# adeebkor/fenicsx-fus

Hardware: AMD Instinct MI355X
Metric: DOF-updates/sec (RK4 step) at p=4 hex fp64 (higher is better)
Workload: dtype f64; 1 GPU; 3D homogeneous wave, hex p=4 f64, Linear RK4, weak scaling: 64^3 cells per GPU (BASELINE.json configs[1]); ndofs_global=16974593, cells_per_gpu=262144, medium=water, partition=x-slabs x1, transport=none, blocks=8192, mfma_contractions=False, mfma_4x4x4_index1=False, packed_fp32=False, lds_bytes_per_block=72504

## Files before the change

fenicsx-fus_amd/csrc/fusmi.hip:

```cpp
#include "../../include/fusmi.h"

#include <dlfcn.h>
#include <hip/hip_runtime.h>
#include <rccl/rccl.h>
#include <limits>

#include <algorithm>
#include <cmath>
#include <cstdio>
#include <cstring>
#include <atomic>
#include <map>
#include <mutex>
#include <tuple>
#include <memory>
#include <string>
#include <vector>

#include "kernels.hpp"
#include "layout.hpp"
#include "tables.hpp"

using namespace fus;

// ... 221 lines not shown
  *p = q;
  return FUS_OK;
}
template <typename U>
static int upload(std::vector<void*>& pool, U** p, const std::vector<U>& v, hipStream_t st)
{
  FUSCHK(dalloc(pool, p, v.size()));
  if (!v.empty())
    HIPCHK(hipMemcpyAsync(*p, v.data(), v.size() * sizeof(U), hipMemcpyHostToDevice, st));
  return FUS_OK;
}
static inline unsigned nblk(int64_t n, int bs = 256) { return (unsigned)((n + bs - 1) / bs); }

struct ProfScope
{
  fus_ctx* c;
  Prof* p = nullptr;
  hipEvent_t e0 = nullptr, e1 = nullptr;
  ProfScope(fus_ctx* c_, const char* name) : c(c_)
  {
    bool take = c->prof == 1;
    if (c->prof == 2 && !strncmp(name, "stiffness", 9))
      take = (c->profs[name].seen++ % c->prof_sample) == 0;
    if (take)
    {
      p = &c->profs[name];
      (void)hipEventCreate(&e0), (void)hipEventCreate(&e1);
      (void)hipEventRecord(e0, c->stream);
    }
  }
  ~ProfScope()
  {
    if (p)
    {
      (void)hipEventRecord(e1, c->stream);
      p->ev.emplace_back(e0, e1);
    }
  }
};

template <typename T, int P, int OP, int ATOMIC, int STAGE, int NF, int GEOM, int TD = 3, int MF = 0, int PK = 0>
static int launch_block_op_v(fus_op* op, const T* geo, const T* coef, const T* x, T* bvec,
                             const StageArgs<T>& S, int blk_begin, int blk_count)
{
  if (blk_count <= 0)
    return FUS_OK;
  constexpr int N = P + 1;
  KArgs<T, N> K;
  for (int i = 0; i < N * N; ++i)
    K.Dk.d[i] = (T)op->D[i], K.Dk.dt[i] = (T)op->D[(i % N) * N + i / N];

  for (int i = 0; i < N; ++i)
    K.Dk.w[i] = (T)op->wts[i], K.Dk.x[i] = (T)op->nodes[i];
  static std::atomic<uint64_t> attr_set{0};
  const uint64_t dev_bit = 1ull << (op->ctx->device & 63);
  if (!(attr_set.load(std::memory_order_relaxed) & dev_bit))
  {
    HIPCHK(hipFuncSetAttribute(reinterpret_cast<const void*>(&k_block_op<T, P, OP, ATOMIC, STAGE, NF, GEOM, TD, MF, PK>),
                               hipFuncAttributeMaxDynamicSharedMemorySize, 160 * 1024));
    attr_set.fetch_or(dev_bit, std::memory_order_relaxed);
  }
  K.A = op->A;
  if (GEOM == GEOM_DIAG)
  {
    for (int q = 0; q < N; ++q)
      for (int i = 0; i < N; ++i)
      {
        double acc = 0;
        for (int m = 0; m < N; ++m)
          acc += op->D[m * N + q] * op->wts[m] * op->D[m * N + i];
        K.Dk.d[q * N + i] = K.Dk.dt[q * N + i] = (T)acc;
      }
  }
  K.A.blk_begin = blk_begin;
  K.A.blk_count = blk_count;
  K.Dg = static_cast<const T*>(op->d_Dg), K.geo = geo, K.coef = coef, K.x = x, K.bvec = bvec;
  K.partial = static_cast<T*>(op->d_partial);
  K.S = S;
  int grid = blk_count;
  if (GEOM != GEOM_STREAM && TD == 3 && op->ctx->walk != 0)
  {
    int per_cu = op->ctx->walk;
    if (per_cu < 0)
    {
      static std::mutex occ_mu;
      static std::map<std::tuple<int, int, size_t>, int> occ_cache;
      int occ = 0;
      {
        std::lock_guard<std::mutex> lk(occ_mu);
        const auto key = std::make_tuple(op->ctx->device, op->L.waves, op->lds_bytes);
        auto it = occ_cache.find(key);
        if (it == occ_cache.end())
        {
          int nb = 0;
          HIPCHK(hipOccupancyMaxActiveBlocksPerMultiprocessor(
              &nb, reinterpret_cast<const void*>(&k_block_op<T, P, OP, ATOMIC, STAGE, NF, GEOM, TD, MF, PK>), 64 * op->L.waves,
              op->lds_bytes));
          it = occ_cache.emplace(key, std::max(nb, 1)).first;
        }
        occ = it->second;
      }
      per_cu = (blk_count >= 4 * occ * op->ctx->num_cus) ? occ : 0;
    }
    if (per_cu > 0)
      grid = std::min(blk_count, per_cu * op->ctx->num_cus);
  }
  hipLaunchKernelGGL((k_block_op<T, P, OP, ATOMIC, STAGE, NF, GEOM, TD, MF, PK>), dim3(grid),
                     dim3(64 * op->L.waves), op->lds_bytes, op->ctx->stream, K);
  HIPCHK(hipGetLastError());
  return FUS_OK;
}

template <typename T, int P, int OP, int STAGE, int NF = 1>
static int launch_block_op(fus_op* op, const T* geo, const T* coef, const T* x, T* bvec,
                           const StageArgs<T>& S, int blk_begin = 0, int blk_count = -1)
{
  if (NF > op->nfields)
    return fail(FUS_ERR_STATE, "operator data was not created for two-field models (option fields=2)");
  if (blk_count < 0)
    blk_count = op->L.nblocks - blk_begin;
  const int b0 = blk_begin, nb = blk_count;
  if constexpr (P >= 8)
  {
    if (op->tdim == 2)
      return op->deterministic
                 ? launch_block_op_v<T, P, OP, 0, STAGE, NF, GEOM_STREAM, 2>(op, geo, coef, x, bvec, S, b0, nb)
                 : launch_block_op_v<T, P, OP, 1, STAGE, NF, GEOM_STREAM, 2>(op, geo, coef, x, bvec, S, b0, nb);
    if (!(op->affine || op->trilinear))
      return op->deterministic
                 ? launch_block_op_v<T, P, OP, 0, STAGE, NF, GEOM_STREAM>(op, geo, coef, x, bvec, S, b0, nb)
                 : launch_block_op_v<T, P, OP, 1, STAGE, NF, GEOM_STREAM>(op, geo, coef, x, bvec, S, b0, nb);
    const T* gc = static_cast<const T*>(op->d_Gc);
    if (op->affine)
      return op->deterministic
                 ? launch_block_op_v<T, P, OP, 0, STAGE, NF, GEOM_AFFINE>(op, gc, coef, x, bvec, S, b0, nb)
                 : launch_block_op_v<T, P, OP, 1, STAGE, NF, GEOM_AFFINE>(op, gc, coef, x, bvec, S, b0, nb);
    return op->deterministic
               ? launch_block_op_v<T, P, OP, 0, STAGE, NF, GEOM_TRILINEAR>(op, gc, coef, x, bvec, S, b0, nb)
               : launch_block_op_v<T, P, OP, 1, STAGE, NF, GEOM_TRILINEAR>(op, gc, coef, x, bvec, S, b0, nb);
  }
  else
  {
  if (op->tdim == 2)
    return op->deterministic
               ? launch_block_op_v<T, P, OP, 0, STAGE, NF, GEOM_STREAM, 2>(op, geo, coef, x, bvec, S, b0, nb)
               : launch_block_op_v<T, P, OP, 1, STAGE, NF, GEOM_STREAM, 2>(op, geo, coef, x, bvec, S, b0, nb);
  if constexpr ((P == 6 || P == 7) && OP == OP_STIFFNESS && (STAGE == STAGE_NONE || STAGE >= 3))
  {
    if (op->mfma && !op->deterministic && op->tdim == 3 && (op->affine || op->trilinear))
    {
      const T* gc = static_cast<const T*>(op->d_Gc);
      return op->affine ? launch_block_op_v<T, P, OP, 1, STAGE, NF, GEOM_AFFINE, 3, 1>(op, gc, coef, x, bvec, S, b0, nb)
                        : launch_block_op_v<T, P, OP, 1, STAGE, NF, GEOM_TRILINEAR, 3, 1>(op, gc, coef, x, bvec, S, b0, nb);
    }
  }
  if constexpr (sizeof(T) == 4 && P >= 5 && P <= 7 && OP == OP_STIFFNESS)
  {
    if (op->pk && !op->mfma && !op->deterministic && op->tdim == 3 && (op->affine || op->trilinear))
    {
      const T* gc = static_cast<const T*>(op->d_Gc);
      return op->affine ? launch_block_op_v<T, P, OP, 1, STAGE, NF, GEOM_AFFINE, 3, 0, 1>(op, gc, coef, x, bvec, S, b0, nb)
                        : launch_block_op_v<T, P, OP, 1, STAGE, NF, GEOM_TRILINEAR, 3, 0, 1>(op, gc, coef, x, bvec, S, b0, nb);
    }
// ... 2439 lines not shown
```

fenicsx-fus_amd/csrc/kernels.hpp:

```cpp
#pragma once
#include <hip/hip_runtime.h>
#include <stdint.h>

#include "geom.hpp"

namespace fus
{

struct ShapeDev
{
  int32_t nelem, nloc, nint, nrounds;
  int64_t rounds_off, ldm_off;
};

struct BlockArgs
{
  const int32_t* blk_shape;
  const ShapeDev* shapes;
  const int32_t* blk_elem_off;
  const int32_t* blk_int_off;
  const int64_t* blk_sh_off;
  const int32_t* sh_gidx;
  const int32_t* sh_ppos;
  const int16_t* rounds;
  const uint16_t* ldm;
  int32_t nblocks;
  int32_t blk_begin;
  int32_t blk_count;
  int32_t lds_nloc;
  int32_t lds_nelem;
  int32_t waves;
};

template <typename T>
struct StageArgs
{
  const T* minv;
  T *vn, *un, *u0, *v0, *u_, *v_;
  T adt, bdt, gval;
  T b0dt, pdt, third;
  const int32_t* blk_bnd_off;
  const int32_t* bnd_idx;
  const T* bnd_src;
  const T* bnd_abs;
  const T* x2;
  const T* coef2;
  const T* bnd_src2;
  T dgval;
  const T* m0;
  const T* mn1;
};

enum
{
  STAGE_NONE = -1
// ... 1937 lines not shown
    const T w = FUS_LD(vn), v = FUS_LD(v0), va = FUS_LD(u_), xs = FUS_LD(un);
    FUS_ST(un, xs + (w * adt - va * R.pdt));
    vnext = kv * adt + v;
    FUS_ST(v_, vnext);
  }
  else if (STAGE == 7)
  {
    const T w = FUS_LD(vn), v = FUS_LD(v0), va = FUS_LD(u_), vb = FUS_LD(v_), xs = FUS_LD(un);
    FUS_ST(u0, (xs - vb * R.pdt) + ((va + vb) * T(2) + (v + w)) * R.b0dt);
    vnext = kv * bdt + ((vb * T(2) + (va + w)) - v) * R.third;
    FUS_ST(v0, vnext);
  }
  else
  {
    const T w = FUS_LD(vn);
    FUS_ST(u_, w * bdt + FUS_LD(u_));
    FUS_ST(v_, kv * bdt + FUS_LD(v_));
    FUS_ST(un, w * adt + FUS_LD(u0));
    vnext = kv * adt + FUS_LD(v0);
    FUS_ST(vn, vnext);
  }
#undef FUS_LD
#undef FUS_ST
  return vnext;
}

template <typename T, int N>
struct KArgs
{
  BlockArgs A;
  DTab<T, N> Dk;
  const T* Dg;
  const T* geo;
  const T* coef;
  const T* x;
  T* bvec;
  T* partial;
  StageArgs<T> S;
};

template <typename T, int N>
__device__ __forceinline__ void load_stage_args(const KArgs<T, N> __attribute__((address_space(4))) * q, StageArgs<T>& S)
{
  S.minv = q->S.minv;
  S.vn = q->S.vn, S.un = q->S.un, S.u0 = q->S.u0, S.v0 = q->S.v0, S.u_ = q->S.u_, S.v_ = q->S.v_;
  S.adt = q->S.adt, S.bdt = q->S.bdt, S.gval = q->S.gval;
  S.b0dt = q->S.b0dt, S.pdt = q->S.pdt, S.third = q->S.third;
  S.blk_bnd_off = q->S.blk_bnd_off, S.bnd_idx = q->S.bnd_idx;
  S.bnd_src = q->S.bnd_src, S.bnd_abs = q->S.bnd_abs;
  S.x2 = q->S.x2, S.coef2 = q->S.coef2, S.bnd_src2 = q->S.bnd_src2, S.dgval = q->S.dgval;
  S.m0 = q->S.m0, S.mn1 = q->S.mn1;
}

template <typename T, int P, int OP, int ATOMIC, int STAGE, int NF, int GEOM, int TD = 3, int MF = 0, int PK = 0>
__global__ void __launch_bounds__((P <= 4) ? 512 : FUS_MID_THREADS, (P >= 8) ? FUS_HI_WAVES : (P <= 4 && is_aff(GEOM))
                                                            ? 4
                                                            : ((GEOM == GEOM_TRILINEAR || (is_aff(GEOM) && P <= 6)) ? FUS_TRI_WAVES_T(T, P) : (FUS_PF1(T, P, OP, ATOMIC, GEOM, TD) ? 2 : 1)))
k_block_op(const KArgs<T, P + 1> kernel_args)
{
  (void)kernel_args;
  static_assert(TD == 3 || GEOM == GEOM_STREAM, "quadrilaterals use the streamed geometry");
  typedef KArgs<T, P + 1> KArgsT;
  typedef DTab<T, P + 1> DTabT;
  static_assert(offsetof(KArgsT, Dk) == sizeof(BlockArgs) && offsetof(DTabT, dt) == sizeof(T) * ((P + 1) * (P + 1) + 2 * (P + 1)),
                "dtab_row reads the table at these kernarg offsets");
  constexpr int N = P + 1, N2 = N * N, Nd = (TD == 3) ? N * N * N : N * N;
  constexpr int EPW = (64 / N2) > 0 ? (64 / N2) : 1;
  constexpr int LPE = (N2 <= 64) ? 64 : 128;
  constexpr int SLOT = tile_slot_entries<T, N, TD>();
  static_assert(N2 <= 128, "degrees up to 10");
  static_assert(LPE == 64 || !MF, "degrees 8-10: no matrix-core variants");
  static_assert(!PK || (sizeof(T) == 4 && EPW == 1 && LPE == 64 && TD == 3 && OP == OP_STIFFNESS && ATOMIC && !MF
                        && GEOM != GEOM_STREAM),
                "packed path: fp32 stiffness, degrees 5-7, per-cell geometry, LDS-atomic accumulation");
  constexpr int EPS = PK ? 2 : 1;

  typedef const KArgs<T, N> __attribute__((address_space(4))) * KP;
#define FUS_KARGS(q)                                                                               \
  KP q = (KP)__builtin_amdgcn_kernarg_segment_ptr();                             \
  asm volatile("" : "+s"(q))
  constexpr int GCS = geom_cell_stride(GEOM);
  constexpr int AW = 8 / (int)sizeof(T);
  typedef double A2 __attribute__((ext_vector_type(2)));
  extern __shared__ __align__(16) unsigned char smem_raw[];
#define FUS_PHASE_LDS(q)                                                                           \
  const int lds_nloc = q->A.lds_nloc, lds_nelem = q->A.lds_nelem, nwaves = q->A.waves;             \
  const int slots = (nwaves * 64 / LPE) * EPW * EPS;                                               \
  T* x_l = reinterpret_cast<T*>(smem_raw);                                                         \
  double* y_l = reinterpret_cast<double*>(x_l + lds_nloc);  \
  T* x2_l = reinterpret_cast<T*>(y_l + lds_nloc);                 \
  T* scratch = x2_l + (NF == 2 ? lds_nloc : 0);                                                    \
  T* D_l = scratch + (size_t)slots * SLOT;        \
  T* cf_l = D_l + N2;                                              \
  T* cf2_l = cf_l + lds_nelem;                                                                     \
  T* gc_l = cf2_l + (NF == 2 ? lds_nelem : 0);  \
  T* w_l = gc_l + GCS * lds_nelem;   \
  T* pt_l = w_l + (N <= 8 ? 8 : 12);                                                               \
  uint16_t* ldm_l = reinterpret_cast<uint16_t*>(w_l + (GCS ? (N <= 8 ? 16 : 24) : 0));  \
  int16_t* rt_l = reinterpret_cast<int16_t*>(ldm_l + (size_t)lds_nelem * Nd);                      \
  (void)y_l, (void)x2_l, (void)scratch, (void)D_l, (void)cf_l, (void)cf2_l, (void)gc_l, (void)w_l, (void)pt_l,      \
      (void)ldm_l, (void)rt_l, (void)slots

  const int tid0 = threadIdx.x, nthr = blockDim.x;
#define FUS_TID()                                                                                  \
  int tid = tid0;                                                                                  \
  asm volatile("" : "+v"(tid))
#define FUS_LANE_COORDS(q)                                                                         \
  FUS_TID();                                                                                       \
  const int lane = tid % LPE, wave = tid / LPE;         \
  const int s = lane / N2, p = lane - s * N2;                                                      \
  const int b = p / N, c = p - b * N;                                                              \
  const bool active = s < EPW;                                                                     \
  const int myslot = (wave * EPW + (active ? s : 0)) * EPS;                                        \
                                \
  T* sA = reinterpret_cast<T*>(smem_raw) + (size_t)((NF == 2 ? 2 : 1) + AW) * q->A.lds_nloc         \
          + (size_t)myslot * SLOT;                                                                 \
  T* sB = sA

  struct Meta
  {
    ShapeDev sh;
    int elem_off, int_off;
    int64_t sh_off;
  };
  auto meta_of = [&](KP q, int bk) -> Meta
  {
    Meta M;
    M.sh = q->A.shapes[q->A.blk_shape[bk]];
    M.elem_off = q->A.blk_elem_off[bk];
    M.int_off = q->A.blk_int_off[bk];
    M.sh_off = q->A.blk_sh_off[bk];
    return M;
  };
  typedef T V2 __attribute__((ext_vector_type(2)));
  typedef uint32_t U4 __attribute__((ext_vector_type(4)));
  constexpr int UI = (P <= 3) ? 3 : ((P == 4) ? 2 : (P <= 6 ? 4 : (P == 7 ? FUS_UI_P7 : FUS_UI_HI))),
                US = (P <= 3) ? 4 : ((P == 4) ? 3 : (P <= 7 ? 5 : FUS_UI_HI)),
                UL = (P <= 3) ? 2 : ((P == 4) ? 1 : 4);
  struct PLoad
  {
    V2 xi[UI], xi2[UI];
    T xs[US], xs2[US];
    U4 lq[UL];
    T cfv, cf2v, gcv, gcv2, dgv, xtail, xtail2;
  };
  auto p_idx = [&](KP q, const Meta& M, bool enable, int (&gi)[US]) __attribute__((always_inline))
  {
    FUS_TID();
    const int nsh = M.sh.nloc - M.sh.nint;
    const int32_t* gix = q->A.sh_gidx + M.sh_off;
#pragma unroll
    for (int u = 0; u < US; ++u)
      gi[u] = (enable && tid + u * nthr < nsh) ? gix[tid + u * nthr] : -1;
  };
  auto p_load = [&](KP q, const Meta& M, PLoad& L, bool with_tables, bool enable, const int (&gi)[US])
      __attribute__((always_inline))
  {
    FUS_TID();
    const ShapeDev& sh = M.sh;
    const T* __restrict__ x = q->x;
    const T* __restrict__ x2 = (NF == 2) ? q->S.x2 : x;
    const T* __restrict__ coef = q->coef;
    const T* __restrict__ coef2 = (NF == 2) ? q->S.coef2 : coef;
    const T* __restrict__ geo = q->geo;
    const T* __restrict__ Dg = q->Dg;
    const V2* xg = reinterpret_cast<const V2*>(x + M.int_off);
    const V2* xg2 = reinterpret_cast<const V2*>(x2 + M.int_off);
    const int nvec = sh.nint >> 1;
    const int nsh = sh.nloc - sh.nint;
    const int32_t* gix = q->A.sh_gidx + M.sh_off;
    const int n16 = (sh.nelem * Nd * 2 + 15) >> 4;
    const U4* lsrc = reinterpret_cast<const U4*>(q->A.ldm + sh.ldm_off);
    const int ngc = sh.nelem * GCS;
#pragma unroll
    for (int u = 0; u < UI; ++u)
    {
      const bool ok = enable && tid + u * nthr < nvec;
      L.xi[u] = ok ? xg[tid + u * nthr] : V2(T(0));
      L.xi2[u] = (NF == 2 && ok) ? xg2[tid + u * nthr] : V2(T(0));
    }
#pragma unroll
    for (int u = 0; u < UL; ++u)
      L.lq[u] = (enable && tid + u * nthr < n16) ? lsrc[tid + u * nthr] : U4(0u);
    L.cfv = (enable && tid < sh.nelem) ? coef[M.elem_off + tid] : T(0);
    L.cf2v = (NF == 2 && enable && tid < sh.nelem) ? coef2[M.elem_off + tid] : T(0);
    L.gcv = (enable && tid < ngc) ? geo[(int64_t)M.elem_off * GCS + tid] : T(0);
    L.gcv2 = (GCS > 7 && enable && tid + nthr < ngc) ? geo[(int64_t)M.elem_off * GCS + tid + nthr] : T(0);
    L.dgv = (with_tables && enable && tid < N2 + 2 * N) ? Dg[tid] : T(0);
    L.xtail = (enable && tid == 0 && (sh.nint & 1)) ? x[M.int_off + sh.nint - 1] : T(0);
    L.xtail2 = (NF == 2 && enable && tid == 0 && (sh.nint & 1)) ? x2[M.int_off + sh.nint - 1] : T(0);
#pragma unroll
    for (int u = 0; u < US; ++u)
    {
      L.xs[u] = gi[u] >= 0 ? x[gi[u]] : T(0);
      L.xs2[u] = (NF == 2 && gi[u] >= 0) ? x2[gi[u]] : T(0);
    }
  };
  auto p_commit = [&](KP q, const Meta& M, const PLoad& L, bool with_tables) __attribute__((always_inline))
  {
    FUS_PHASE_LDS(q);
    FUS_TID();
    const ShapeDev& sh = M.sh;
    const T* __restrict__ x = q->x;
    const T* __restrict__ x2 = (NF == 2) ? q->S.x2 : x;
    const T* __restrict__ coef = q->coef;
    const T* __restrict__ coef2 = (NF == 2) ? q->S.coef2 : coef;
    const T* __restrict__ geo = q->geo;
    const T* __restrict__ Dg = q->Dg;
    const V2* xg = reinterpret_cast<const V2*>(x + M.int_off);
    const V2* xg2 = reinterpret_cast<const V2*>(x2 + M.int_off);
    const int nvec = sh.nint >> 1;
    const int nsh = sh.nloc - sh.nint;
    const int32_t* gix = q->A.sh_gidx + M.sh_off;
    const int n16 = (sh.nelem * Nd * 2 + 15) >> 4;
    const U4* lsrc = reinterpret_cast<const U4*>(q->A.ldm + sh.ldm_off);
    const int ngc = sh.nelem * GCS;
    for (int i = tid; i < (sh.nloc + 1) / 2; i += nthr)
      reinterpret_cast<A2*>(y_l)[i] = A2(0.0);
#pragma unroll
    for (int u = 0; u < UI; ++u)
      if (tid + u * nthr < nvec)
      {
        reinterpret_cast<V2*>(x_l)[tid + u * nthr] = L.xi[u];
        if (NF == 2)
          reinterpret_cast<V2*>(x2_l)[tid + u * nthr] = L.xi2[u];
      }
#pragma unroll
    for (int u = 0; u < UL; ++u)
      if (tid + u * nthr < n16)
        reinterpret_cast<U4*>(ldm_l)[tid + u * nthr] = L.lq[u];
    if (tid < sh.nelem)
    {
      cf_l[tid] = L.cfv;
      if (NF == 2)
        cf2_l[tid] = L.cf2v;
    }
    if (tid < ngc)
      gc_l[tid] = L.gcv;
    if (GCS > 7 && tid + nthr < ngc)
      gc_l[tid + nthr] = L.gcv2;
    if (with_tables)
    {
      if (tid < N2)
        D_l[tid] = L.dgv;
      if (GCS && tid >= N2 && tid < N2 + N)
        w_l[tid - N2] = L.dgv;
      if (GCS && tid >= N2 + N && tid < N2 + 2 * N)
        pt_l[tid - N2 - N] = L.dgv;
      for (int k = tid + nthr; k < N2 + 2 * N; k += nthr)
      {
        const T v = Dg[k];
        if (k < N2)
          D_l[k] = v;
        else if (GCS && k < N2 + N)
          w_l[k - N2] = v;
        else if (GCS)
          pt_l[k - N2 - N] = v;
      }
    }
    if (tid == 0 && (sh.nint & 1))
    {
      x_l[sh.nint - 1] = L.xtail;
      if (NF == 2)
        x2_l[sh.nint - 1] = L.xtail2;
    }
#pragma unroll
    for (int u = 0; u < US; ++u)
      if (tid + u * nthr < nsh)
      {
        x_l[sh.nint + tid + u * nthr] = L.xs[u];
        if (NF == 2)
          x2_l[sh.nint + tid + u * nthr] = L.xs2[u];
      }
    constexpr int UB = 8;
    for (int base = tid + UI * nthr; base < nvec; base += nthr * UB)
    {
      V2 v[UB], v2[UB];
#pragma unroll
      for (int u = 0; u < UB; ++u)
        if (base + u * nthr < nvec)
        {
          v[u] = xg[base + u * nthr];
          if (NF == 2)
            v2[u] = xg2[base + u * nthr];
        }
#pragma unroll
      for (int u = 0; u < UB; ++u)
        if (base + u * nthr < nvec)
        {
          reinterpret_cast<V2*>(x_l)[base + u * nthr] = v[u];
          if (NF == 2)
            reinterpret_cast<V2*>(x2_l)[base + u * nthr] = v2[u];
        }
    }
    for (int base = tid + US * nthr; base < nsh; base += nthr * UB)
    {
      int g[UB];
      T v[UB], v2[UB];
#pragma unroll
      for (int u = 0; u < UB; ++u)
        g[u] = (base + u * nthr < nsh) ? gix[base + u * nthr] : 0;
#pragma unroll
      for (int u = 0; u < UB; ++u)
      {
        v[u] = x[g[u]];
        if (NF == 2)
          v2[u] = x2[g[u]];
      }
#pragma unroll
      for (int u = 0; u < UB; ++u)
        if (base + u * nthr < nsh)
        {
          x_l[sh.nint + base + u * nthr] = v[u];
          if (NF == 2)
            x2_l[sh.nint + base + u * nthr] = v2[u];
        }
    }
    for (int base = tid + UL * nthr; base < n16; base += nthr * UB)
    {
      U4 q[UB];
#pragma unroll
      for (int u = 0; u < UB; ++u)
        if (base + u * nthr < n16)
          q[u] = lsrc[base + u * nthr];
#pragma unroll
      for (int u = 0; u < UB; ++u)
        if (base + u * nthr < n16)
          reinterpret_cast<U4*>(ldm_l)[base + u * nthr] = q[u];
    }
    for (int k = tid + nthr; k < sh.nelem; k += nthr)
    {
      cf_l[k] = coef[M.elem_off + k];
      if (NF == 2)
        cf2_l[k] = coef2[M.elem_off + k];
    }
    for (int k = tid + (GCS > 7 ? 2 : 1) * nthr; k < ngc; k += nthr)
      gc_l[k] = geo[(int64_t)M.elem_off * GCS + k];
    if (!ATOMIC)
      for (int k = tid; k < sh.nrounds * slots; k += nthr)
        rt_l[k] = q->A.rounds[sh.rounds_off + k];
  };

  FUS_KARGS(q0);
  const int blk_end = q0->A.blk_begin + q0->A.blk_count;
  const int blk_stride = gridDim.x;
  int wg = blockIdx.x;
  if (FUS_XCD_REMAP)
  {
    const int G = gridDim.x, q8 = G >> 3, r8 = G & 7, xc = wg & 7;
    wg = xc * q8 + (xc < r8 ? xc : r8) + (wg >> 3);
  }
  int blk = wg + q0->A.blk_begin;
  FUS_STAMP(blk, 0);
  ElemIn<T, N, OP, GEOM, TD> inA, inB;
  auto first_fetch = [&](KP q, const Meta& Mm) __attribute__((always_inline))
  {
    FUS_LANE_COORDS(q);
    (void)b, (void)c, (void)sA, (void)sB;
    const int slots = (q->A.waves * 64 / LPE) * EPW * EPS;
    const int nt0 = ATOMIC ? (Mm.sh.nelem + slots - 1) / slots : Mm.sh.nrounds;
    int e0 = -1;
    if (active && nt0 > 0)
      e0 = ATOMIC ? (myslot < Mm.sh.nelem ? myslot : -1) : (int)q->A.rounds[Mm.sh.rounds_off + myslot];
    elem_fetch<T, N, OP, GEOM, TD>(inA, e0, q->geo, Mm.elem_off, p);
  };
  PLoad L;
  {
    const Meta M0 = meta_of(q0, blk);
    first_fetch(q0, M0);
    int gi0[US];
    p_idx(q0, M0, true, gi0);
    p_load(q0, M0, L, true, true, gi0);
  }
  bool first = true;
  for (;;)
  {
  FUS_KARGS(qc);
  FUS_PHASE_LDS(qc);
  FUS_LANE_COORDS(qc);
  const Meta M = meta_of(qc, blk);
  const ShapeDev& sh = M.sh;
  const int elem_off = M.elem_off;
  const int ntrips = ATOMIC ? (sh.nelem + slots - 1) / slots : sh.nrounds;
  auto elem_of = [&](int r) -> int
  {
    if (!active || r >= ntrips)
      return -1;
    if (ATOMIC)
      return (r * slots + myslot < sh.nelem) ? r * slots + myslot : -1;
    return (int)rt_l[r * slots + myslot];
  };
#ifdef FUS_PROBE_PFREE
  if (first)
    p_commit(qc, M, L, true);
  else
  {
    FUS_TID();
    for (int i = tid; i < (M.sh.nloc + 1) / 2; i += nthr)
      reinterpret_cast<A2*>(y_l)[i] = A2(0.0);
  }
#else
  p_commit(qc, M, L, first);
#endif
  const int blk_next = blk + blk_stride;
  const bool has_next = blk_next < blk_end;
  constexpr bool IDX_EARLY = false;
  int gi_n[US];
  if constexpr (IDX_EARLY)
  {
    Meta Mi{};
    if (has_next)
      Mi = meta_of(qc, blk_next);
    p_idx(qc, Mi, has_next, gi_n);
  }
  __syncthreads();
  FUS_STAMP(blk, 1);
#ifdef FUS_STAGGER
  if (tid0 >= 256)
    __builtin_amdgcn_s_sleep(FUS_STAGGER);
#endif
  T Drb[N], Drc[N], Dcb[N], Dcc[N], w3[N];
  T wbc, pb, pc;
  {
#pragma unroll
    for (int j = 0; j < N; ++j)
    {
      constexpr bool inreg = (OP == OP_STIFFNESS) && !(FUS_PF1(T, P, OP, ATOMIC, GEOM, TD) && P >= 6)
                             && GEOM != GEOM_TRILINEAR && GEOM != GEOM_DIAG && !(is_aff(GEOM) && (P == 5 || P == 6)) && !MF;
      Drb[j] = inreg ? D_l[b * N + j] : T(0);
      Drc[j] = inreg ? D_l[c * N + j] : T(0);
      Dcb[j] = inreg ? D_l[j * N + b] : T(0);
      Dcc[j] = inreg ? D_l[j * N + c] : T(0);
    }
#pragma unroll
    for (int a = 0; a < N; ++a)
      w3[a] = (GEOM == GEOM_AFFINE) ? w_l[a] * w_l[b] * w_l[c] : T(0);
    wbc = (GEOM == GEOM_TRILINEAR || GEOM == GEOM_DIAG) ? w_l[b] * w_l[c] : T(0);
    pb = (GEOM == GEOM_TRILINEAR) ? pt_l[b] : T(0), pc = (GEOM == GEOM_TRILINEAR) ? pt_l[c] : T(0);
  }

  FUS_KARGS(qt);
  DTab<T, N> Dk;
  if constexpr (!dtab_by_rows<T, N>())
  {
#pragma unroll
    for (int i = 0; i < N * N; ++i)
      Dk.d[i] = qt->Dk.d[i];
  }
#pragma unroll
  for (int i = 0; i < N; ++i)
    Dk.w[i] = qt->Dk.w[i], Dk.x[i] = qt->Dk.x[i];
  const T* __restrict__ geo = qt->geo;
#define FUS_ELEM_COMPUTE(in)                                                                       \
  do                                                                                               \
  {                                                                                                \
    if constexpr (LPE == 128 && TD == 2)                                                           \
      elem_compute2d<T, N, OP, ATOMIC, NF, true>(in, Drb, Drc, Dcb, Dcc, x_l, y_l, sA, ldm_l,      \
                                                 cf_l, x2_l, cf2_l, p, b, c, s == 0);              \
// ... 28 lines not shown
    {
      int li[N];
      T F0[N], F1[N], F2[N];
      constexpr int DL = (P >= 6) ? 1 : 0;
      const bool act = elem_stiff_fwd<T, N, NF, DL>(inA, Dk, Drb, Drc, D_l, x_l, sA, ldm_l, cf_l, x2_l, cf2_l, p, b,
                                                    c, li, F0, F1, F2);
      elem_fetch<T, N, OP, GEOM, TD>(inA, elem_of(r + 1), geo, elem_off, p);
      if (act)
        elem_stiff_bwd<T, N, DL, ATOMIC>(Dk, Dcb, Dcc, D_l, y_l, sA, p, b, c, li, F0, F1, F2);
      if (!ATOMIC && nwaves > 1)
        __syncthreads();
    }
  }
  else
  for (int r = 0; r < ntrips; r += 2)
  {
    const bool has1 = r + 1 < ntrips;
    elem_fetch<T, N, OP, GEOM, TD>(inB, elem_of(r + 1), geo, elem_off, p);
    FUS_ELEM_COMPUTE(inA);
    if (r == 0)
      FUS_STAMP(blk, 5);
    if (r == 2)
      FUS_STAMP(blk, 7);
    if (!ATOMIC && nwaves > 1)
      __syncthreads();
    elem_fetch<T, N, OP, GEOM, TD>(inA, elem_of(r + 2), geo, elem_off, p);
    if (has1)
    {
      FUS_ELEM_COMPUTE(inB);
      if (r == 0)
        FUS_STAMP(blk, 6);
      if (!ATOMIC && nwaves > 1)
        __syncthreads();
    }
  }
#undef FUS_ELEM_COMPUTE
  {
  FUS_KARGS(qe);
  FUS_PHASE_LDS(qe);
  FUS_TID();
  const Meta M = meta_of(qe, blk);
  const ShapeDev& sh = M.sh;
  const int int_off = M.int_off;
  const int64_t sh_off = M.sh_off;
  StageArgs<T> S;
  load_stage_args<T, N>(qe, S);
  T* __restrict__ bvec = qe->bvec;
  T* __restrict__ partial = qe->partial;
  const int32_t* __restrict__ pp = qe->A.sh_ppos + sh_off;
  const int nsh = sh.nloc - sh.nint;
  int ppv[US];
#pragma unroll
  for (int u = 0; u < US; ++u)
    ppv[u] = (tid + u * nthr < nsh) ? pp[tid + u * nthr] : -1;

  const int nvec = sh.nint >> 1;
    constexpr bool EPI2 = (P <= 4) && (NF == 1);
    struct Epi
    {
      bool on;
      int i, o;
      V2 bv, mi, w, a0, b0, au, av, m1, m0v, us;
    };
    auto epi_load = [&](int i, Epi& E, int part) __attribute__((always_inline))
    {
      if (part != 2)
      {
      E.on = i < nvec;
      E.i = i, E.o = int_off + 2 * i;
      E.bv = E.mi = E.w = E.a0 = E.b0 = E.au = E.av = E.m1 = E.m0v = E.us = V2(T(0));
#ifdef FUS_PROBE_EFREE
      auto ld = [&](const T* ptr) -> V2 { return E.on ? V2(T(1)) + V2(T((uintptr_t)ptr & 7)) : V2(T(0)); };
#else
      auto ld = [&](const T* ptr) -> V2
      { return E.on ? __builtin_nontemporal_load(reinterpret_cast<const V2*>(ptr + E.o)) : V2(T(0)); };
#endif
      constexpr bool WV = NF == 2;
      if (STAGE == 0)
        E.a0 = ld(S.u0), E.b0 = ld(S.v0);
      else if (STAGE == 4)
        E.b0 = ld(S.v0);
      else
        E.w = ld(S.vn);
      if (WV && S.mn1)
        E.m1 = ld(S.mn1), E.m0v = ld(S.m0);
      else
        E.mi = ld(S.minv);
      if (STAGE == 3)
        E.au = ld(S.u_), E.av = ld(S.v_);
      else if (STAGE == 1)
        E.au = ld(S.u_), E.av = ld(S.v_), E.a0 = ld(S.u0), E.b0 = ld(S.v0);
      else if (STAGE == 5)
        E.b0 = ld(S.v0);
      else if (STAGE == 6)
        E.b0 = ld(S.v0), E.au = ld(S.u_);
      else if (STAGE == 7)
        E.b0 = ld(S.v0), E.au = ld(S.u_), E.av = ld(S.v_);
      }
      if (part != 1)
      {
        constexpr bool WV2 = NF == 2;
        const A2 a2 = E.on ? reinterpret_cast<const A2*>(y_l)[E.i] : A2(0.0);
        E.bv = V2{(T)a2[0], (T)a2[1]};
        if ((WV2 && S.mn1) || STAGE >= 4)
          E.us = E.on ? reinterpret_cast<const V2*>(x_l)[E.i] : V2(T(0));
      }
    };
    auto epi_store = [&](const Epi& E) __attribute__((always_inline))
    {
      if (!E.on)
        return;
      auto st = [&](T* ptr, V2 val) { __builtin_nontemporal_store(val, reinterpret_cast<V2*>(ptr + E.o)); };
      V2 kv;
      if (NF == 2 && S.mn1)
      {
        const V2 vs = stage_is_first(STAGE) ? E.b0 : E.w;
        kv = (E.bv - E.m1 * vs * vs) / (E.m0v + E.m1 * E.us);
      }
      else
        kv = E.bv * E.mi;
      if (STAGE == 0)
      {
        st(S.u_, E.b0 * S.bdt + E.a0);
        st(S.v_, kv * S.bdt + E.b0);
        st(S.un, E.b0 * S.adt + E.a0);
        st(S.vn, kv * S.adt + E.b0);
      }
      else if (STAGE == 4)
      {
        st(S.un, E.b0 * S.adt + E.us);
        st(S.v_, kv * S.adt + E.b0);
      }
      else if (STAGE == 3)
      {
        st(S.u0, E.w * S.bdt + E.au);
        st(S.v0, kv * S.bdt + E.av);
      }
      else if (STAGE == 5)
      {
        st(S.un, E.us + (E.w * S.adt - E.b0 * S.pdt));
        st(S.v_, kv * S.adt + E.b0);
      }
      else if (STAGE == 6)
      {
        st(S.un, E.us + (E.w * S.adt - E.au * S.pdt));
        st(S.v_, kv * S.adt + E.b0);
      }
      else if (STAGE == 7)
      {
        st(S.u0, (E.us - E.av * S.pdt) + ((E.au + E.av) * T(2) + (E.b0 + E.w)) * S.b0dt);
        st(S.v0, kv * S.bdt + ((E.av * T(2) + (E.au + E.w)) - E.b0) * S.third);
      }
      else
      {
        st(S.u_, E.w * S.bdt + E.au);
        st(S.v_, kv * S.bdt + E.av);
        st(S.un, E.w * S.adt + E.a0);
        st(S.vn, kv * S.adt + E.b0);
      }
    };
    constexpr int EPIU = EPI2 ? 2 : epiu_of<T>(P, GEOM, NF);
    constexpr bool EARLY = epi_early<T>(P);
    Epi Ef[EPIU];
    if (EARLY && STAGE != STAGE_NONE)
    {
#pragma unroll
      for (int u = 0; u < EPIU; ++u)
        epi_load(tid + u * nthr, Ef[u], 1);
    }
  __syncthreads();
  FUS_STAMP(blk, 2);

  {
    FUS_KARGS(qn);
    Meta Mn{};
    if (has_next)
      Mn = meta_of(qn, blk_next);
#ifdef FUS_PROBE_PFREE
    if constexpr (!IDX_EARLY)
      p_idx(qn, Mn, false, gi_n);
    p_load(qn, Mn, L, false, false, gi_n);
#else
    if constexpr (!IDX_EARLY)
      p_idx(qn, Mn, has_next, gi_n);
    p_load(qn, Mn, L, false, has_next, gi_n);
#endif
  }
  if (STAGE == STAGE_NONE)
  {
    V2* bg = reinterpret_cast<V2*>(bvec + int_off);
    for (int i = tid; i < nvec; i += nthr)
    {
      const A2 a2 = reinterpret_cast<const A2*>(y_l)[i];
      bg[i] = V2{(T)a2[0], (T)a2[1]};
    }
    if (tid == 0 && (sh.nint & 1))
      bvec[int_off + sh.nint - 1] = (T)y_l[sh.nint - 1];
  }
  else
  {
    const int k0 = S.blk_bnd_off[blk], k1 = S.blk_bnd_off[blk + 1];
    if (k1 > k0)
    {
      const T* vstage = stage_is_first(STAGE) ? S.v0 : S.vn;
      for (int k = k0 + tid; k < k1; k += nthr)
      {
        const int gi = S.bnd_idx[k];
        T add = S.gval * S.bnd_src[k] - S.bnd_abs[k] * vstage[gi];
        if (NF == 2)
          add += S.dgval * S.bnd_src2[k];
        y_l[gi - int_off] += add;
      }
      __syncthreads();
    }
    if (tid == 0 && (sh.nint & 1))
      (void)stage_update_dof<T, STAGE>((int64_t)int_off + sh.nint - 1, (T)y_l[sh.nint - 1], S.minv, S.vn, S.un, S.u0,
                                       S.v0, S.u_, S.v_, S.adt, S.bdt, (NF == 2) ? S.m0 : nullptr,
                                       (NF == 2) ? S.mn1 : nullptr, LeanRK<T>{S.b0dt, S.pdt, S.third});
#pragma unroll
    for (int u = 0; u < EPIU; ++u)
      epi_load(tid + u * nthr, Ef[u], EARLY ? 2 : 0);
#pragma unroll
    for (int u = 0; u < EPIU; ++u)
      epi_store(Ef[u]);
    for (int i = tid + EPIU * nthr; i < nvec; i += EPIU * nthr)
    {
      Epi E[EPIU];
#pragma unroll
      for (int u = 0; u < EPIU; ++u)
        epi_load(i + u * nthr, E[u], 0);
#pragma unroll
      for (int u = 0; u < EPIU; ++u)
        epi_store(E[u]);
    }
  }
#pragma unroll
  for (int u = 0; u < US; ++u)
    if (ppv[u] >= 0)
      partial[ppv[u]] = (T)y_l[sh.nint + tid + u * nthr];
  for (int k = tid + US * nthr; k < nsh; k += nthr)
    partial[pp[k]] = (T)y_l[sh.nint + k];
  }
  FUS_TRACE_END(blk);
  if (!has_next)
    break;
  __syncthreads();
  blk = blk_next;
  first = false;
  {
    FUS_KARGS(qf);
    const Meta Mf = meta_of(qf, blk);
    first_fetch(qf, Mf);
  }
  }
#undef FUS_KARGS
#undef FUS_LANE_COORDS
#undef FUS_PHASE_LDS
#undef FUS_TID
}


template <typename T, typename I>
__global__ void k_shared_reduce(int64_t s0, int64_t s1, const I* __restrict__ sh_ptr,
                                const I* __restrict__ sh_pairs, const T* __restrict__ partial,
                                T* __restrict__ bsh)
{
  const int64_t s = s0 + (int64_t)blockIdx.x * blockDim.x + threadIdx.x;
  if (s >= s1)
    return;
  T acc = T(0);
  for (I k = sh_ptr[s]; k < sh_ptr[s + 1]; ++k)
    acc += partial[sh_pairs[k]];
  bsh[s] = acc;
}

template <typename T>
struct BndNext
{
  int enabled;
  int32_t npairs;
  const T *srcw, *absw, *src2w;
  T gnext, dgnext;
  T* partial;
};

template <typename T>
__device__ __forceinline__ void boundary_next(const BndNext<T>& B, int32_t last_pair, T vnext)
{
  if (B.enabled && last_pair >= B.npairs)
  {
    const int32_t k = last_pair - B.npairs;
    T v = B.gnext * B.srcw[k] - B.absw[k] * vnext;
    if (B.src2w)
      v += B.dgnext * B.src2w[k];
    B.partial[last_pair] = v;
  }
}



constexpr int FUS_MAX_PLANES = 16;
struct PartialPlanes
{
  int32_t bnd0;
  int32_t cnt[FUS_MAX_PLANES];
  int32_t off[FUS_MAX_PLANES];
};

template <typename T, int STAGE>
__global__ void __launch_bounds__(256)
k_shared_stage_planes(int64_t n, const PartialPlanes PL, const uint64_t* __restrict__ bnd_mask,
// ... 401 lines not shown
```

Before: 13.90 billion DOF-updates/s.

## Add WALK template specialization to slim single-block kernel path

Adds a WALK template parameter to the block operator kernel and picks the walking (persistent, multi-block) variant only when the grid is smaller than the block count. The non-walking variant drops the next-block prefetch and the compiler barriers on the kernarg pointer and thread id. It also uses predicated loads with 32-bit offset addressing and wave-uniform guards on the tail loops. The aim is to cut register pressure, scalar and address arithmetic, and dead prefetch code when each workgroup handles one block. The cost is twice as many kernel instantiations and more complex load-guard logic.

```diff
diff --git a/fenicsx-fus_amd/csrc/fusmi.hip b/fenicsx-fus_amd/csrc/fusmi.hip
--- a/fenicsx-fus_amd/csrc/fusmi.hip
+++ b/fenicsx-fus_amd/csrc/fusmi.hip
@@ -297,14 +297,6 @@
 
   for (int i = 0; i < N; ++i)
     K.Dk.w[i] = (T)op->wts[i], K.Dk.x[i] = (T)op->nodes[i];
-  static std::atomic<uint64_t> attr_set{0};
-  const uint64_t dev_bit = 1ull << (op->ctx->device & 63);
-  if (!(attr_set.load(std::memory_order_relaxed) & dev_bit))
-  {
-    HIPCHK(hipFuncSetAttribute(reinterpret_cast<const void*>(&k_block_op<T, P, OP, ATOMIC, STAGE, NF, GEOM, TD, MF, PK>),
-                               hipFuncAttributeMaxDynamicSharedMemorySize, 160 * 1024));
-    attr_set.fetch_or(dev_bit, std::memory_order_relaxed);
-  }
   K.A = op->A;
   if (GEOM == GEOM_DIAG)
   {
@@ -322,8 +314,9 @@
   K.Dg = static_cast<const T*>(op->d_Dg), K.geo = geo, K.coef = coef, K.x = x, K.bvec = bvec;
   K.partial = static_cast<T*>(op->d_partial);
   K.S = S;
+  constexpr bool CAN_WALK = GEOM != GEOM_STREAM && TD == 3;
   int grid = blk_count;
-  if (GEOM != GEOM_STREAM && TD == 3 && op->ctx->walk != 0)
+  if (CAN_WALK && op->ctx->walk != 0)
   {
     int per_cu = op->ctx->walk;
     if (per_cu < 0)
@@ -339,8 +332,8 @@
         {
           int nb = 0;
           HIPCHK(hipOccupancyMaxActiveBlocksPerMultiprocessor(
-              &nb, reinterpret_cast<const void*>(&k_block_op<T, P, OP, ATOMIC, STAGE, NF, GEOM, TD, MF, PK>), 64 * op->L.waves,
-              op->lds_bytes));
+              &nb, reinterpret_cast<const void*>(&k_block_op<T, P, OP, ATOMIC, STAGE, NF, GEOM, TD, MF, PK, CAN_WALK ? 1 : 0>),
+              64 * op->L.waves, op->lds_bytes));
           it = occ_cache.emplace(key, std::max(nb, 1)).first;
         }
         occ = it->second;
@@ -350,10 +343,27 @@
     if (per_cu > 0)
       grid = std::min(blk_count, per_cu * op->ctx->num_cus);
   }
-  hipLaunchKernelGGL((k_block_op<T, P, OP, ATOMIC, STAGE, NF, GEOM, TD, MF, PK>), dim3(grid),
-                     dim3(64 * op->L.waves), op->lds_bytes, op->ctx->stream, K);
-  HIPCHK(hipGetLastError());
-  return FUS_OK;
+  auto launch = [&](auto walk) -> int
+  {
+    constexpr int WALK = decltype(walk)::value;
+    const auto kernel = &k_block_op<T, P, OP, ATOMIC, STAGE, NF, GEOM, TD, MF, PK, WALK>;
+    static std::atomic<uint64_t> attr_set{0};
+    const uint64_t dev_bit = 1ull << (op->ctx->device & 63);
+    if (!(attr_set.load(std::memory_order_relaxed) & dev_bit))
+    {
+      HIPCHK(hipFuncSetAttribute(reinterpret_cast<const void*>(kernel), hipFuncAttributeMaxDynamicSharedMemorySize,
+                                 160 * 1024));
+      attr_set.fetch_or(dev_bit, std::memory_order_relaxed);
+    }
+    hipLaunchKernelGGL((k_block_op<T, P, OP, ATOMIC, STAGE, NF, GEOM, TD, MF, PK, WALK>), dim3(grid),
+                       dim3(64 * op->L.waves), op->lds_bytes, op->ctx->stream, K);
+    HIPCHK(hipGetLastError());
+    return FUS_OK;
+  };
+  if constexpr (CAN_WALK)
+    if (grid < blk_count)
+      return launch(std::integral_constant<int, 1>{});
+  return launch(std::integral_constant<int, 0>{});
 }
 
 template <typename T, int P, int OP, int STAGE, int NF = 1>
diff --git a/fenicsx-fus_amd/csrc/kernels.hpp b/fenicsx-fus_amd/csrc/kernels.hpp
--- a/fenicsx-fus_amd/csrc/kernels.hpp
+++ b/fenicsx-fus_amd/csrc/kernels.hpp
@@ -1,6 +1,7 @@
 #pragma once
 #include <hip/hip_runtime.h>
 #include <stdint.h>
+#include <type_traits>
 
 #include "geom.hpp"
 
@@ -2044,7 +2045,7 @@
   S.m0 = q->S.m0, S.mn1 = q->S.mn1;
 }
 
-template <typename T, int P, int OP, int ATOMIC, int STAGE, int NF, int GEOM, int TD = 3, int MF = 0, int PK = 0>
+template <typename T, int P, int OP, int ATOMIC, int STAGE, int NF, int GEOM, int TD = 3, int MF = 0, int PK = 0, int WALK = 0>
 __global__ void __launch_bounds__((P <= 4) ? 512 : FUS_MID_THREADS, (P >= 8) ? FUS_HI_WAVES : (P <= 4 && is_aff(GEOM))
                                                             ? 4
                                                             : ((GEOM == GEOM_TRILINEAR || (is_aff(GEOM) && P <= 6)) ? FUS_TRI_WAVES_T(T, P) : (FUS_PF1(T, P, OP, ATOMIC, GEOM, TD) ? 2 : 1)))
@@ -2069,8 +2070,9 @@
 
   typedef const KArgs<T, N> __attribute__((address_space(4))) * KP;
 #define FUS_KARGS(q)                                                                               \
-  KP q = (KP)__builtin_amdgcn_kernarg_segment_ptr();                             \
-  asm volatile("" : "+s"(q))
+  KP q = (KP)__builtin_amdgcn_kernarg_segment_ptr();                                               \
+  if constexpr (WALK)                                                                              \
+    asm volatile("" : "+s"(q))
   constexpr int GCS = geom_cell_stride(GEOM);
   constexpr int AW = 8 / (int)sizeof(T);
   typedef double A2 __attribute__((ext_vector_type(2)));
@@ -2096,7 +2098,8 @@
   const int tid0 = threadIdx.x, nthr = blockDim.x;
 #define FUS_TID()                                                                                  \
   int tid = tid0;                                                                                  \
-  asm volatile("" : "+v"(tid))
+  if constexpr (WALK)                                                                              \
+    asm volatile("" : "+v"(tid))
 #define FUS_LANE_COORDS(q)                                                                         \
   FUS_TID();                                                                                       \
   const int lane = tid % LPE, wave = tid / LPE;         \
@@ -2115,8 +2118,11 @@
     int elem_off, int_off;
     int64_t sh_off;
   };
+  Meta Mone{};
   auto meta_of = [&](KP q, int bk) -> Meta
   {
+    if constexpr (!WALK)
+      return Mone;
     Meta M;
     M.sh = q->A.shapes[q->A.blk_shape[bk]];
     M.elem_off = q->A.blk_elem_off[bk];
@@ -2124,6 +2130,21 @@
     M.sh_off = q->A.blk_sh_off[bk];
     return M;
   };
+  auto at32 = [](auto* base, int i) -> auto&
+  {
+    typedef std::remove_reference_t<decltype(*base)> E;
+    typedef std::conditional_t<std::is_const_v<E>, const char, char> C;
+    return *reinterpret_cast<E*>(reinterpret_cast<C*>(base) + (uint32_t)i * (uint32_t)sizeof(E));
+  };
+#define FUS_UNIFORM(cond) (WALK || __builtin_amdgcn_readfirstlane((int)(cond)))
+#define FUS_STAGE_LD(dst, cond, expr, fill)                                                        \
+  do                                                                                               \
+  {                                                                                                \
+    if constexpr (WALK)                                                                            \
+      dst = (cond) ? (expr) : (fill);                                                              \
+    else if (cond)                                                                                 \
+      dst = (expr);                                                                                \
+  } while (0)
   typedef T V2 __attribute__((ext_vector_type(2)));
   typedef uint32_t U4 __attribute__((ext_vector_type(4)));
   constexpr int UI = (P <= 3) ? 3 : ((P == 4) ? 2 : (P <= 6 ? 4 : (P == 7 ? FUS_UI_P7 : FUS_UI_HI))),
@@ -2143,7 +2164,7 @@
     const int32_t* gix = q->A.sh_gidx + M.sh_off;
 #pragma unroll
     for (int u = 0; u < US; ++u)
-      gi[u] = (enable && tid + u * nthr < nsh) ? gix[tid + u * nthr] : -1;
+      FUS_STAGE_LD(gi[u], enable && tid + u * nthr < nsh, at32(gix, tid + u * nthr), -1);
   };
   auto p_load = [&](KP q, const Meta& M, PLoad& L, bool with_tables, bool enable, const int (&gi)[US])
       __attribute__((always_inline))
@@ -2168,24 +2189,28 @@
     for (int u = 0; u < UI; ++u)
     {
       const bool ok = enable && tid + u * nthr < nvec;
-      L.xi[u] = ok ? xg[tid + u * nthr] : V2(T(0));
-      L.xi2[u] = (NF == 2 && ok) ? xg2[tid + u * nthr] : V2(T(0));
+      FUS_STAGE_LD(L.xi[u], ok, at32(xg, tid + u * nthr), V2(T(0)));
+      FUS_STAGE_LD(L.xi2[u], NF == 2 && ok, at32(xg2, tid + u * nthr), V2(T(0)));
     }
 #pragma unroll
     for (int u = 0; u < UL; ++u)
-      L.lq[u] = (enable && tid + u * nthr < n16) ? lsrc[tid + u * nthr] : U4(0u);
-    L.cfv = (enable && tid < sh.nelem) ? coef[M.elem_off + tid] : T(0);
-    L.cf2v = (NF == 2 && enable && tid < sh.nelem) ? coef2[M.elem_off + tid] : T(0);
-    L.gcv = (enable && tid < ngc) ? geo[(int64_t)M.elem_off * GCS + tid] : T(0);
-    L.gcv2 = (GCS > 7 && enable && tid + nthr < ngc) ? geo[(int64_t)M.elem_off * GCS + tid + nthr] : T(0);
-    L.dgv = (with_tables && enable && tid < N2 + 2 * N) ? Dg[tid] : T(0);
-    L.xtail = (enable && tid == 0 && (sh.nint & 1)) ? x[M.int_off + sh.nint - 1] : T(0);
-    L.xtail2 = (NF == 2 && enable && tid == 0 && (sh.nint & 1)) ? x2[M.int_off + sh.nint - 1] : T(0);
+      FUS_STAGE_LD(L.lq[u], enable && tid + u * nthr < n16, at32(lsrc, tid + u * nthr), U4(0u));
+    const T* cfg = coef + M.elem_off;
+    const T* cfg2 = coef2 + M.elem_off;
+    const T* gcg = geo + (int64_t)M.elem_off * GCS;
+    FUS_STAGE_LD(L.cfv, enable && tid < sh.nelem, at32(cfg, tid), T(0));
+    FUS_STAGE_LD(L.cf2v, NF == 2 && enable && tid < sh.nelem, at32(cfg2, tid), T(0));
+    FUS_STAGE_LD(L.gcv, enable && tid < ngc, at32(gcg, tid), T(0));
+    FUS_STAGE_LD(L.gcv2, GCS > 7 && enable && tid + nthr < ngc, at32(gcg, tid + nthr), T(0));
+    FUS_STAGE_LD(L.dgv, with_tables && enable && tid < N2 + 2 * N, at32(Dg, tid), T(0));
+    FUS_STAGE_LD(L.xtail, enable && tid == 0 && (sh.nint & 1), x[M.int_off + sh.nint - 1], T(0));
+    FUS_STAGE_LD(L.xtail2, NF == 2 && enable && tid == 0 && (sh.nint & 1), x2[M.int_off + sh.nint - 1], T(0));
 #pragma unroll
     for (int u = 0; u < US; ++u)
     {
-      L.xs[u] = gi[u] >= 0 ? x[gi[u]] : T(0);
-      L.xs2[u] = (NF == 2 && gi[u] >= 0) ? x2[gi[u]] : T(0);
+      const bool oks = WALK ? gi[u] >= 0 : tid + u * nthr < nsh;
+      FUS_STAGE_LD(L.xs[u], oks, x[(uint32_t)gi[u]], T(0));
+      FUS_STAGE_LD(L.xs2[u], NF == 2 && oks, x2[(uint32_t)gi[u]], T(0));
     }
   };
   auto p_commit = [&](KP q, const Meta& M, const PLoad& L, bool with_tables) __attribute__((always_inline))
@@ -2239,6 +2264,7 @@
         w_l[tid - N2] = L.dgv;
       if (GCS && tid >= N2 + N && tid < N2 + 2 * N)
         pt_l[tid - N2 - N] = L.dgv;
+      if (FUS_UNIFORM(nthr < N2 + 2 * N))
       for (int k = tid + nthr; k < N2 + 2 * N; k += nthr)
       {
         const T v = Dg[k];
@@ -2265,6 +2291,7 @@
           x2_l[sh.nint + tid + u * nthr] = L.xs2[u];
       }
     constexpr int UB = 8;
+    if (FUS_UNIFORM(UI * nthr < nvec))
     for (int base = tid + UI * nthr; base < nvec; base += nthr * UB)
     {
       V2 v[UB], v2[UB];
@@ -2285,6 +2312,7 @@
             reinterpret_cast<V2*>(x2_l)[base + u * nthr] = v2[u];
         }
     }
+    if (FUS_UNIFORM(US * nthr < nsh))
     for (int base = tid + US * nthr; base < nsh; base += nthr * UB)
     {
       int g[UB];
@@ -2308,6 +2336,7 @@
             x2_l[sh.nint + base + u * nthr] = v2[u];
         }
     }
+    if (FUS_UNIFORM(UL * nthr < n16))
     for (int base = tid + UL * nthr; base < n16; base += nthr * UB)
     {
       U4 q[UB];
@@ -2320,12 +2349,14 @@
         if (base + u * nthr < n16)
           reinterpret_cast<U4*>(ldm_l)[base + u * nthr] = q[u];
     }
+    if (FUS_UNIFORM(nthr < sh.nelem))
     for (int k = tid + nthr; k < sh.nelem; k += nthr)
     {
       cf_l[k] = coef[M.elem_off + k];
       if (NF == 2)
         cf2_l[k] = coef2[M.elem_off + k];
     }
+    if (FUS_UNIFORM((GCS > 7 ? 2 : 1) * nthr < ngc))
     for (int k = tid + (GCS > 7 ? 2 : 1) * nthr; k < ngc; k += nthr)
       gc_l[k] = geo[(int64_t)M.elem_off * GCS + k];
     if (!ATOMIC)
@@ -2358,6 +2389,13 @@
   };
   PLoad L;
   {
+    if constexpr (!WALK)
+    {
+      Mone.sh = q0->A.shapes[q0->A.blk_shape[blk]];
+      Mone.elem_off = q0->A.blk_elem_off[blk];
+      Mone.int_off = q0->A.blk_int_off[blk];
+      Mone.sh_off = q0->A.blk_sh_off[blk];
+    }
     const Meta M0 = meta_of(q0, blk);
     first_fetch(q0, M0);
     int gi0[US];
@@ -2395,7 +2433,7 @@
   p_commit(qc, M, L, first);
 #endif
   const int blk_next = blk + blk_stride;
-  const bool has_next = blk_next < blk_end;
+  const bool has_next = WALK && blk_next < blk_end;
   constexpr bool IDX_EARLY = false;
   int gi_n[US];
   if constexpr (IDX_EARLY)
@@ -2530,14 +2568,14 @@
   int ppv[US];
 #pragma unroll
   for (int u = 0; u < US; ++u)
-    ppv[u] = (tid + u * nthr < nsh) ? pp[tid + u * nthr] : -1;
+    FUS_STAGE_LD(ppv[u], tid + u * nthr < nsh, at32(pp, tid + u * nthr), -1);
 
   const int nvec = sh.nint >> 1;
     constexpr bool EPI2 = (P <= 4) && (NF == 1);
     struct Epi
     {
       bool on;
-      int i, o;
+      int i;
       V2 bv, mi, w, a0, b0, au, av, m1, m0v, us;
     };
     auto epi_load = [&](int i, Epi& E, int part) __attribute__((always_inline))
@@ -2545,37 +2583,41 @@
       if (part != 2)
       {
       E.on = i < nvec;
-      E.i = i, E.o = int_off + 2 * i;
-      E.bv = E.mi = E.w = E.a0 = E.b0 = E.au = E.av = E.m1 = E.m0v = E.us = V2(T(0));
+      E.i = i;
+      if constexpr (WALK)
+        E.bv = E.mi = E.w = E.a0 = E.b0 = E.au = E.av = E.m1 = E.m0v = E.us = V2(T(0));
 #ifdef FUS_PROBE_EFREE
-      auto ld = [&](const T* ptr) -> V2 { return E.on ? V2(T(1)) + V2(T((uintptr_t)ptr & 7)) : V2(T(0)); };
+      auto ld = [&](V2& dst, const T* ptr) { dst = E.on ? V2(T(1)) + V2(T((uintptr_t)ptr & 7)) : V2(T(0)); };
 #else
-      auto ld = [&](const T* ptr) -> V2
-      { return E.on ? __builtin_nontemporal_load(reinterpret_cast<const V2*>(ptr + E.o)) : V2(T(0)); };
+      auto ld = [&](V2& dst, const T* ptr)
+      {
+        FUS_STAGE_LD(dst, E.on, __builtin_nontemporal_load(&at32(reinterpret_cast<const V2*>(ptr + int_off), E.i)),
+                     V2(T(0)));
+      };
 #endif
       constexpr bool WV = NF == 2;
       if (STAGE == 0)
-        E.a0 = ld(S.u0), E.b0 = ld(S.v0);
+        ld(E.a0, S.u0), ld(E.b0, S.v0);
       else if (STAGE == 4)
-        E.b0 = ld(S.v0);
+        ld(E.b0, S.v0);
       else
-        E.w = ld(S.vn);
+        ld(E.w, S.vn);
       if (WV && S.mn1)
-        E.m1 = ld(S.mn1), E.m0v = ld(S.m0);
+        ld(E.m1, S.mn1), ld(E.m0v, S.m0);
       else
-        E.mi = ld(S.minv);
+        ld(E.mi, S.minv);
       if (STAGE == 3)
-        E.au = ld(S.u_), E.av = ld(S.v_);
+        ld(E.au, S.u_), ld(E.av, S.v_);
       else if (STAGE == 1)
-        E.au = ld(S.u_), E.av = ld(S.v_), E.a0 = ld(S.u0), E.b0 = ld(S.v0);
+        ld(E.au, S.u_), ld(E.av, S.v_), ld(E.a0, S.u0), ld(E.b0, S.v0);
       else if (STAGE == 5)
-        E.b0 = ld(S.v0);
+        ld(E.b0, S.v0);
       else if (STAGE == 6)
-        E.b0 = ld(S.v0), E.au = ld(S.u_);
+        ld(E.b0, S.v0), ld(E.au, S.u_);
       else if (STAGE == 7)
-        E.b0 = ld(S.v0), E.au = ld(S.u_), E.av = ld(S.v_);
-      }
-      if (part != 1)
+        ld(E.b0, S.v0), ld(E.au, S.u_), ld(E.av, S.v_);
+      }
+      if (part != 1 && (WALK || E.on))
       {
         constexpr bool WV2 = NF == 2;
         const A2 a2 = E.on ? reinterpret_cast<const A2*>(y_l)[E.i] : A2(0.0);
@@ -2588,7 +2630,8 @@
     {
       if (!E.on)
         return;
-      auto st = [&](T* ptr, V2 val) { __builtin_nontemporal_store(val, reinterpret_cast<V2*>(ptr + E.o)); };
+      auto st = [&](T* ptr, V2 val)
+      { __builtin_nontemporal_store(val, &at32(reinterpret_cast<V2*>(ptr + int_off), E.i)); };
       V2 kv;
       if (NF == 2 && S.mn1)
       {
@@ -2649,6 +2692,7 @@
   __syncthreads();
   FUS_STAMP(blk, 2);
 
+  if constexpr (WALK)
   {
     FUS_KARGS(qn);
     Meta Mn{};
@@ -2701,6 +2745,7 @@
 #pragma unroll
     for (int u = 0; u < EPIU; ++u)
       epi_store(Ef[u]);
+    if (FUS_UNIFORM(EPIU * nthr < nvec))
     for (int i = tid + EPIU * nthr; i < nvec; i += EPIU * nthr)
     {
       Epi E[EPIU];
@@ -2714,8 +2759,9 @@
   }
 #pragma unroll
   for (int u = 0; u < US; ++u)
-    if (ppv[u] >= 0)
-      partial[ppv[u]] = (T)y_l[sh.nint + tid + u * nthr];
+    if (WALK ? ppv[u] >= 0 : tid + u * nthr < nsh)
+      partial[(uint32_t)ppv[u]] = (T)y_l[sh.nint + tid + u * nthr];
+  if (FUS_UNIFORM(US * nthr < nsh))
   for (int k = tid + US * nthr; k < nsh; k += nthr)
     partial[pp[k]] = (T)y_l[sh.nint + k];
   }
@@ -2735,6 +2781,8 @@
 #undef FUS_LANE_COORDS
 #undef FUS_PHASE_LDS
 #undef FUS_TID
+#undef FUS_STAGE_LD
+#undef FUS_UNIFORM
 }
 
 
```

Result: faster. 14.97 billion DOF-updates/s, median of 6 (+7.7%).
